# cggos/ptam_cg

Measured on AMD Instinct MI355X. Metric: BA LM iterations/s (50 KF x 5k pts) [+ tracked frames/s @640x480 in 'tracking'], higher is better.
Workload: dtype f64; 1 GPU; bundle_50kf_x_5000pts_dense; keyframes=50, points_total=5000, measurements_total=250000, measurements_rank0=250000, estimator=Tukey, parallelism=1 GPU, halfsample=R

## Files before the change

ptam_cg_amd/csrc/ldlt_chain.inc:

```
struct ChainLds {
    double PF[2][2][NB][6];
    double T0[NB * LDP];
    double T1[NB * LDP];
    double T2[NB * LDP];
    double T3[NB * LDP];
    double T4[NB * LDP];
    double iD[NB], Dv[NB], z[NB];
    double zp[8][NB];
    int one_xcd;
    int staged[2];
};
#define CH_TS (NB * LDP)
#define CH_MAX_NB 28
#define CH_LDS_MAX (160 * 1024)
__host__ __device__ __forceinline__ size_t ch_lds_bytes(int band) { return sizeof(ChainLds) + 8 + (size_t)(band + 1) * CH_TS * sizeof(double); }
#define CH_BW_SL 12
__host__ __device__ __forceinline__ size_t ch_lds_bytes_bw(int band, int nblk) {
    const size_t rhs = (size_t)(2 + CH_BW_SL) * nblk * NB + NB, tiles = (size_t)(band + 1) * CH_TS;
    return sizeof(ChainLds) + 8 + (rhs > tiles ? rhs : tiles) * sizeof(double);
}
#define CH_BW_MAXT 9

__device__ __forceinline__ double ch_ld(const double* p) {
    return __longlong_as_double(__hip_atomic_load((const long long*)p, __ATOMIC_RELAXED, __HIP_MEMORY_SCOPE_AGENT));
}
__device__ __forceinline__ void ch_st(double* p, double v, bool one_xcd) {
    if (one_xcd)
        *p = v;
    else
        __hip_atomic_store((long long*)p, __double_as_longlong(v), __ATOMIC_RELAXED, __HIP_MEMORY_SCOPE_AGENT);
}
__device__ __forceinline__ void ch_ld2_issue(double2& v, const double2* p) { asm volatile("global_load_dwordx4 %0, %1, off sc1" : "=v"(v) : "v"(p) : "memory"); }
__device__ __forceinline__ void ch_ld2_wait() { asm volatile("s_waitcnt vmcnt(0)" ::: "memory"); }
__device__ __forceinline__ void ch_raise(unsigned* f, unsigned seq, bool one_xcd) {
    const unsigned v = (seq << 1) | (one_xcd ? 1u : 0u);
    if (one_xcd)
        asm volatile("global_store_dword %0, %1, off" ::"v"(f), "v"(v) : "memory");
    else
        __hip_atomic_store(f, v, __ATOMIC_RELAXED, __HIP_MEMORY_SCOPE_AGENT);
}
__device__ __forceinline__ unsigned ch_flag(const unsigned* f) { return __hip_atomic_load(f, __ATOMIC_RELAXED, __HIP_MEMORY_SCOPE_AGENT); }
__device__ __forceinline__ unsigned ch_wait(const unsigned* f, unsigned seq, unsigned* err, int limit) {
    int spins = 0;
    unsigned v;
    while (((v = ch_flag(f)) >> 1) != seq) {
        __builtin_amdgcn_s_sleep(1);
        if (++spins > limit || ((spins & 255) == 0 && ch_flag(err) == seq)) {
            __hip_atomic_store(err, seq, __ATOMIC_RELAXED, __HIP_MEMORY_SCOPE_AGENT);
            break;
        }
    }
    return v;
}
__device__ __forceinline__ void ch_wait_lanes(const unsigned* f, bool active, unsigned seq, unsigned* err, int limit) {
    int spins = 0;
    for (;;) {
        const bool up = !active || (ch_flag(f) >> 1) == seq;
        if (__builtin_amdgcn_ballot_w64(!up) == 0) break;
        __builtin_amdgcn_s_sleep(1);
        if (++spins > limit || ((spins & 255) == 0 && ch_flag(err) == seq)) {
            __hip_atomic_store(err, seq, __ATOMIC_RELAXED, __HIP_MEMORY_SCOPE_AGENT);
            break;
        }
    }
}
__host__ __device__ __forceinline__ int ch_roles(int nblk) { return nblk > 2 ? nblk : 2; }
__host__ __device__ __forceinline__ size_t ch_flag_words(int nblk, int band) { return 2 + 3 * (size_t)nblk + (size_t)nblk * (band + 1); }

struct ChainArgs {
    double *S, *E, *L, *Dg, *y;
    unsigned* flags;
    int k0, k1, kr, n;
};
__global__ void __launch_bounds__(TPB, 2) ldlt_chain_kernel(BaDev d, ChainArgs a0, ChainArgs a1, int clubs, int cur, int do_bw) {
    const int club = ((int)(blockIdx.x & 7) - d.chain_xcd) & 7;
    if (club >= clubs) return;
    const ChainArgs& a = club == 0 ? a0 : a1;
    const int k0 = a.k0, k1 = a.k1, kr = a.kr;
    const int role = blockIdx.x >> 3;
    if (role == 0 && club == 0) { TL_MARK(d, 9) }
    extern __shared__ __attribute__((aligned(16))) double ch_lds[];
    ChainLds& s = *(ChainLds*)ch_lds;
    const int band = se_band(d), nblk = d.npad / NB;
    const int n_roles = ch_roles(kr - k0);
    if (role >= n_roles) return;
    const unsigned seq = d.solve_seq;
    unsigned* const err = d.sflags;
    unsigned* const F = a.flags + 1;
    unsigned* const RF = F + nblk;
    unsigned* const XCC = RF + nblk;
    unsigned* const XFb = XCC + nblk + 1;
    auto XF = [&](int r, int m) { return XFb + (size_t)r * (band + 1) + (m - max(0, r - band)); };
    double* __restrict__ S = a.S;
    double* __restrict__ E = a.E;
    double* __restrict__ Lf = a.L;
    const int tid = threadIdx.x;
    const int w = __builtin_amdgcn_readfirstlane(tid >> 6), lane = tid & 63;
    const int qi = w >> 1, qj = w & 1;
    const int i16 = lane & 15, m4 = lane >> 4;
    const int colq = 16 * qj + i16;
    const unsigned my_xcc = __builtin_amdgcn_s_getreg(20 | (0 << 6) | (3 << 11)) & 0xf;
    if (tid == 0) __hip_atomic_store(XCC + role, (seq << 4) | my_xcc, __ATOMIC_RELAXED, __HIP_MEMORY_SCOPE_AGENT);
    auto mma_t = [&](const double* A, const double (&bt)[NB / 4]) {
        v4f64 acc = {0, 0, 0, 0};
        const double* pa = A + (16 * qi + i16) * LDP + m4;
        double a8[NB / 4];
#pragma unroll
        for (int kk = 0; kk < NB / 4; kk++) a8[kk] = pa[4 * kk];
#pragma unroll
        for (int kk = 0; kk < NB / 4; kk++) acc = __builtin_amdgcn_mfma_f64_16x16x4f64(a8[kk], bt[kk], acc, 0, 0, 0);
        return acc;
    };
#ifdef K7_TIMING
    int nst_ = 0;
#define CH_STAMP() if (role == 0 && threadIdx.x == 192 && nst_ < 200) d.dbg[32 + nst_++] = (long long)__builtin_readcyclecounter();
#define CH_SEEN(t_) if (lane == 0) d.dbg[440 + k] = d.dbg[456 + k] = 100 + (t_);
#define CH_RT(slot) d.dbg[600 + (slot)] = (long long)__builtin_amdgcn_s_memrealtime();
#else
#define CH_STAMP()
#define CH_SEEN(t_)
#define CH_RT(slot)
#endif
    if (role == 0) {
        const double e0 = m4 == 0 ? 1.0 : 0.0, e1 = m4 == 1 ? 1.0 : 0.0, e2 = m4 == 2 ? 1.0 : 0.0, e3 = m4 == 3 ? 1.0 : 0.0;
        v4f64 accK;
#pragma unroll
        for (int v = 0; v < 4; v++) {
            const int row = 16 * qi + m4 + 4 * v;
            accK[v] = S[se_blk(k0, k0, band) + max(row, colq) * NB + min(row, colq)];
        }
        bool one_xcd = false;
        for (int k = k0; k < k1; k++) {
            v4f64 accI;
            const int niter = (min(NB, a.n - k * NB) + 3) / 4;
            if (tid < NB) {
                s.iD[tid] = 1.0;
                s.Dv[tid] = 1.0;
            }
            const int r = k + 1;
            const bool have_row = r < kr;
            const size_t o_rk = have_row ? se_blk(r, k, band) : 0, o_rr = have_row ? se_blk(r, r, band) : 0;
            if (tid < 2) s.staged[tid] = 0;
            int stage_state = have_row ? 0 : 2;
            double stg[2][NB * NB / 64];
            CH_STAMP()
            if (tid == 0) { CH_RT(4 * k + 3) }
#ifdef FL_NO_STAGE
#define FL_STAGE_ON false
#else
#define FL_STAGE_ON true
#endif
#define FACTOR_IDLE_HOOK(t_)                                                                                         \
    if (FL_STAGE_ON && stage_state < 2) {                                                                            \
        if (stage_state == 0 && (r < k0 + 2 || (ch_flag(RF + r) >> 1) == seq)) {                                     \
            _Pragma("unroll") for (int u = 0; u < NB * NB / 64; u++) stg[0][u] = ch_ld(S + o_rk + lane + 64 * u);    \
            _Pragma("unroll") for (int u = 0; u < NB * NB / 64; u++) stg[1][u] = ch_ld(S + o_rr + lane + 64 * u);    \
            stage_state = (t_) + 1 < niter ? 1 : 3;                                                                  \
            CH_SEEN(t_)                                                                                              \
        } else if (stage_state == 1)                                                                                 \
            stage_state = 3;                                                                                         \
        if (stage_state == 3) {                                                                                      \
            _Pragma("unroll") for (int u = 0; u < NB * NB / 64; u++) {                                               \
                const int e_ = lane + 64 * u;                                                                        \
                s.T3[(e_ / NB) * LDP + e_ % NB] = stg[0][u];                                                         \
                s.T4[(e_ / NB) * LDP + e_ % NB] = stg[1][u];                                                         \
            }                                                                                                        \
            if (lane == 0) s.staged[0] = s.staged[1] = 1;                                                            \
            stage_state = 2;                                                                                         \
        }                                                                                                            \
    }
#include "ldlt_factor2.inc"
#undef FACTOR_IDLE_HOOK
            CH_STAMP()
            if (k == k0) {
                if (w == 0) {
                    bool same = true;
                    for (int i = lane; i < n_roles; i += 64) same = same && ch_flag(XCC + i) == ((seq << 4) | my_xcc);
                    const bool all_same = __builtin_amdgcn_ballot_w64(!same) == 0;
                    if (lane == 0) s.one_xcd = all_same;
                }
                __syncthreads();
                one_xcd = s.one_xcd != 0;
            }
            const size_t o_kk = se_blk(k, k, band);
#pragma unroll
            for (int v = 0; v < 4; v++)
                s.T0[(16 * qi + m4 + 4 * v) * LDP + fl_colI] = accI[v];
            auto store_diag = [&]() {
#pragma unroll
                for (int v = 0; v < 4; v++) ch_st(Lf + o_kk + (16 * qi + m4 + 4 * v) * NB + fl_colI, accI[v], one_xcd);
                if (tid < NB) ch_st(a.Dg + k * NB + tid, s.Dv[tid], one_xcd);
            };
            if (!have_row) {
                store_diag();
                asm volatile("s_waitcnt vmcnt(0)" ::: "memory");
                __syncthreads();
                if (tid == 0) ch_raise(F + k, seq, one_xcd);
                break;
            }
            double aop[NB / 4];
            v4f64 accN;
            if (!(s.staged[0] && s.staged[1])) {
                if (r >= k0 + 2 && lane == 0) ch_wait(RF + r, seq, err, d.spin_limit);
                double t3[NB * NB / TPB], t4[NB * NB / TPB];
#pragma unroll
                for (int u = 0; u < NB * NB / TPB; u++) t3[u] = ch_ld(S + o_rk + tid + u * TPB);
#pragma unroll
                for (int u = 0; u < NB * NB / TPB; u++) t4[u] = ch_ld(S + o_rr + tid + u * TPB);
#pragma unroll
                for (int u = 0; u < NB * NB / TPB; u++) {
                    const int e = tid + u * TPB;
                    s.T3[(e / NB) * LDP + e % NB] = t3[u];
                    s.T4[(e / NB) * LDP + e % NB] = t4[u];
                }
                __syncthreads();
            }
#pragma unroll
            for (int kk = 0; kk < NB / 4; kk++) aop[kk] = s.T3[(16 * qi + i16) * LDP + 4 * kk + m4];
#pragma unroll
            for (int v = 0; v < 4; v++) {
                const int row = 16 * qi + m4 + 4 * v;
                accN[v] = s.T4[max(row, colq) * LDP + min(row, colq)];
            }
            CH_STAMP()
            __syncthreads();
            v4f64 x = {0, 0, 0, 0};
            {
                const double* pb = s.T0 + m4 * LDP + colq;
                double b8[NB / 4];
#pragma unroll
                for (int kk = 0; kk < NB / 4; kk++) b8[kk] = pb[4 * kk * LDP];
#pragma unroll
                for (int kk = 0; kk < NB / 4; kk++) x = __builtin_amdgcn_mfma_f64_16x16x4f64(aop[kk], b8[kk], x, 0, 0, 0);
            }
            const double idc = s.iD[colq];
            __builtin_amdgcn_sched_barrier(0);
            store_diag();
            __builtin_amdgcn_sched_barrier(0);
            double lv[4];
#pragma unroll
            for (int v = 0; v < 4; v++) {
                const int e = (16 * qi + m4 + 4 * v);
                lv[v] = x[v] * idc;
                s.T1[e * LDP + colq] = x[v];
                s.T2[e * LDP + colq] = lv[v];
            }
            __syncthreads();
            double bt[NB / 4];
#pragma unroll
            for (int kk = 0; kk < NB / 4; kk++) bt[kk] = s.T2[(16 * qj + i16) * LDP + 4 * kk + m4];
            const v4f64 upd = mma_t(s.T1, bt);
            __builtin_amdgcn_sched_barrier(0);
#pragma unroll
            for (int v = 0; v < 4; v++) ch_st(Lf + o_rk + (16 * qi + m4 + 4 * v) * NB + colq, lv[v], one_xcd);
            __builtin_amdgcn_sched_barrier(0);
#pragma unroll
            for (int v = 0; v < 4; v++) accK[v] = accN[v] - upd[v];
            asm volatile("s_waitcnt vmcnt(0)" ::: "memory");
            __syncthreads();
            if (tid == 0) {
                ch_raise(F + k, seq, one_xcd);
                ch_raise(XF(r, k), seq, one_xcd);
                CH_RT(4 * k)
            }
            if (r == k1) {
                if (w != 1) {
#pragma unroll
                    for (int v = 0; v < 4; v++) S[o_rr + (16 * qi + m4 + 4 * v) * NB + colq] = accK[v];
                }
                break;
            }
            CH_STAMP()
        }
        return;
    }
    if (role == n_roles - 1) {
        double* const bb = ch_lds + (sizeof(ChainLds) + 7) / 8;
        const int b0 = k0 * NB;
        for (int i = k0 * NB + tid; i < kr * NB; i += TPB) bb[i - b0] = E[i];
        __syncthreads();
        const int q = tid & (NB - 1), part = tid >> 5;
        const int row = tid >> 3, g = tid & 7;
        for (int m = k0; m < k1; m++) {
            if (lane == 0) (void)ch_wait(F + m, seq, err, d.spin_limit);
            const size_t o_mm = se_blk(m, m, band);
            double t4[NB / 8];
#pragma unroll
            for (int j = 0; j < NB / 8; j++) t4[j] = ch_ld(Lf + o_mm + (part + 8 * j) * NB + q);
            double p = 0;
#pragma unroll
            for (int j = 0; j < NB / 8; j++) p += t4[j] * bb[m * NB - b0 + part + 8 * j];
            s.zp[part][q] = p;
            __syncthreads();
            if (tid < NB) {
                const double z = ((s.zp[0][tid] + s.zp[1][tid]) + (s.zp[2][tid] + s.zp[3][tid])) +
                                 ((s.zp[4][tid] + s.zp[5][tid]) + (s.zp[6][tid] + s.zp[7][tid]));
                s.z[tid] = z;
                a.y[m * NB + tid] = z;
                if (do_bw) bb[m * NB - b0 + tid] = z / ch_ld(a.Dg + m * NB + tid);
            }
            __syncthreads();
            double zr[NB / 8];
#pragma unroll
            for (int jj = 0; jj < NB / 8; jj++) zr[jj] = s.z[g + 8 * jj];
            const int jhi = min(kr - 1, m + band);
            {
                const int jw = m + 1 + lane;
                ch_wait_lanes(XF(min(jw, jhi), m), jw <= jhi && jhi > m, seq, err, d.spin_limit);
            }
            for (int jb = m + 1; jb <= jhi; jb += 4) {
                const int nj = min(4, jhi - jb + 1);
                double lv[4][NB / 8];
#pragma unroll
                for (int u = 0; u < 4; u++)
                    if (u < nj) {
                        const double* Lj = Lf + se_blk(jb + u, m, band) + row * NB + g;
#pragma unroll
                        for (int jj = 0; jj < NB / 8; jj++) lv[u][jj] = ch_ld(Lj + 8 * jj);
                    }
#pragma unroll
                for (int u = 0; u < 4; u++)
                    if (u < nj) {
                        double sum = 0;
#pragma unroll
                        for (int jj = 0; jj < NB / 8; jj++) sum += lv[u][jj] * zr[jj];
                        sum += dpp_row_shr_f64<1>(sum);
                        sum += dpp_row_shr_f64<2>(sum);
                        sum += dpp_row_shr_f64<4>(sum);
                        if (g == 7) bb[(jb + u) * NB - b0 + row] -= sum;
                    }
            }
            __syncthreads();
        }
        for (int i = k1 * NB + tid; i < kr * NB; i += TPB) E[i] = bb[i - b0];
        if (!do_bw) return;
        {
            const int nrow = kr * NB;
            double* const xs = bb + nrow;
            double* const pend = xs + nrow;
            for (int i = tid; i < CH_BW_SL * nrow; i += TPB) pend[i] = 0.0;
            const int hh = lane >> 5, c32 = lane & (NB - 1);
            const int g4 = lane >> 4, cp = lane & 15;
            constexpr int TW = 3;
            static_assert(3 * TW >= CH_BW_MAXT, "three tile waves cover a block row");
            static_assert(CH_BW_SL == 12, "a slice per tile wave and lane group");
            const int tw = w - 1;
            double* const dstage0 = s.T1;
            static_assert(4 * NB * LDP >= 2 * NB * 34, "the diagonal tiles' staging areas");
            auto stage_diag = [&](int k) {
                const double2* dk = (const double2*)(Lf + se_blk(k, k, band)) + lane;
                double2 dq[3];
#pragma unroll
                for (int i = 0; i < 3; i++)
                    if (tw + 3 * i < NB / 4) ch_ld2_issue(dq[i], dk + 64 * (tw + 3 * i));
                ch_ld2_wait();
                double* const ds = dstage0 + (k & 1) * (NB * 34);
#pragma unroll
                for (int i = 0; i < 3; i++)
                    if (tw + 3 * i < NB / 4) *(double2*)(ds + (4 * (tw + 3 * i) + g4) * 34 + 2 * cp) = dq[i];
            };
            if (w > 0) stage_diag(kr - 1);
            __syncthreads();
#ifdef K7_TIMING
#define BWI_STAMP(i_) if (lane == 0 && w < 2) d.dbg[1400 + 8 * k + 4 * w + (i_)] = (long long)__builtin_readcyclecounter();
            if (tid == 0) d.dbg[1399] = (long long)__builtin_readcyclecounter();
#else
#define BWI_STAMP(i_)
#endif
#pragma unroll 1
            for (int k = kr - 1; k >= 0; k--) {
                const int jb0 = max(0, k - band), nt = k - jb0;
                BWI_STAMP(0)
                double2 lt[TW][NB / 4];
                if (w == 0) {
                    const double* pk = pend + k * NB + c32;
                    const double v = bb[k * NB + c32] - ((((pk[0] + pk[nrow]) + (pk[2 * nrow] + pk[3 * nrow])) + ((pk[4 * nrow] + pk[5 * nrow]) + (pk[6 * nrow] + pk[7 * nrow]))) +
                                                         ((pk[8 * nrow] + pk[9 * nrow]) + (pk[10 * nrow] + pk[11 * nrow])));
                    if (hh == 0) s.z[c32] = v;
                    __builtin_amdgcn_fence(__ATOMIC_RELEASE, "wavefront");
                    __builtin_amdgcn_wave_barrier();
                    double tk[NB / 2], zk[NB / 2];
#pragma unroll
                    for (int u = 0; u < NB / 2; u++) tk[u] = dstage0[(k & 1) * (NB * 34) + c32 * 34 + 16 * hh + u], zk[u] = s.z[16 * hh + u];
                    double p4[4] = {0, 0, 0, 0};
#pragma unroll
                    for (int u = 0; u < NB / 2; u++) p4[u & 3] += (16 * hh + u >= c32) ? tk[u] * zk[u] : 0.0;
                    const double p = (p4[0] + p4[1]) + (p4[2] + p4[3]);
                    const unsigned long long pb_ = (unsigned long long)__double_as_longlong(p);
                    const auto lo_ = __builtin_amdgcn_permlane32_swap((unsigned)pb_, (unsigned)pb_, false, false);
                    const auto hi_ = __builtin_amdgcn_permlane32_swap((unsigned)(pb_ >> 32), (unsigned)(pb_ >> 32), false, false);
                    const double p_up = __longlong_as_double((long long)(((unsigned long long)hi_[1] << 32) | lo_[1]));
                    if (hh == 0) xs[k * NB + c32] = p + p_up;
                    BWI_STAMP(1)
                } else {
                    const double2* src = (const double2*)(Lf + se_blk(k, jb0, band)) + lane;
#pragma unroll
                    for (int i = 0; i < TW; i++)
                        if (tw + 3 * i < nt) {
#pragma unroll
                            for (int u = 0; u < NB / 4; u++) ch_ld2_issue(lt[i][u], src + (size_t)(tw + 3 * i) * (NB * NB / 2) + 64 * u);
                        }
                    if (k > 0)
                        stage_diag(k - 1);
                    else
                        ch_ld2_wait();
                }
                BWI_STAMP(2)
                __syncthreads();
                BWI_STAMP(3)
                if (w > 0) {
                    double xv[NB / 4];
#pragma unroll
                    for (int u = 0; u < NB / 4; u++) xv[u] = xs[k * NB + 4 * u + g4];
                    double* const pslot = pend + (4 * tw + g4) * nrow + jb0 * NB + 2 * cp;
#pragma unroll
                    for (int i = 0; i < TW; i++)
                        if (tw + 3 * i < nt) {
                            double a0 = 0, a1 = 0;
#pragma unroll
                            for (int u = 0; u < NB / 4; u++) a0 += lt[i][u].x * xv[u], a1 += lt[i][u].y * xv[u];
                            __hip_atomic_fetch_add(pslot + (tw + 3 * i) * NB, a0, __ATOMIC_RELAXED, __HIP_MEMORY_SCOPE_WORKGROUP);
                            __hip_atomic_fetch_add(pslot + (tw + 3 * i) * NB + 1, a1, __ATOMIC_RELAXED, __HIP_MEMORY_SCOPE_WORKGROUP);
                        }
                }
                __syncthreads();
            }
            __syncthreads();
            for (int i = tid; i < nrow; i += TPB) d.da[i] = xs[i];
            for (int c2 = tid; c2 < d.C; c2 += TPB) {
                const int f = d.cam_free[c2];
                const double* T = d.pose[cur] + 12 * c2;
                double* Tn = d.pose[cur ^ 1] + 12 * c2;
                double Tl[12], o[12];
#pragma unroll
                for (int i = 0; i < 12; i++) Tl[i] = T[i];
                if (f < 0) {
#pragma unroll
                    for (int i = 0; i < 12; i++) Tn[i] = Tl[i];
                } else {
                    double mu[6];
#pragma unroll
                    for (int i = 0; i < 6; i++) mu[i] = xs[6 * f + i];
                    se3_exp_mul(mu, Tl, o);
#pragma unroll
                    for (int i = 0; i < 12; i++) Tn[i] = o[i];
                }
            }
#ifdef K7_TIMING
            if (tid == 0) d.dbg[1398] = (long long)__builtin_readcyclecounter();
#endif
            if (tid < 64) {
                double sq = 0;
                for (int i = tid; i < min(nrow, d.n); i += 64) sq += xs[i] * xs[i];
                sq = wave_sum_f64(sq);
                if (tid == 0) {
                    d.sumsq2[0] = sq;
                    d.sumsq2[1] = 0.0;
                    if (ch_flag(err) != 0) {
                        d.sc->solve_fault = 1;
                        __hip_atomic_store(err, 0u, __ATOMIC_RELAXED, __HIP_MEMORY_SCOPE_AGENT);
                    }
                }
            }
        }
        return;
    }
    const int r = k0 + role + 1;
    if (r >= kr) return;
    const int j0 = max(k0, r - band), nt = r - j0 + 1;
    double* const tiles = ch_lds + (sizeof(ChainLds) + 7) / 8;
    for (int t = 0; t < nt; t++) {
        const size_t o = se_blk(r, j0 + t, band);
        double v4[NB * NB / TPB];
#pragma unroll
        for (int u = 0; u < NB * NB / TPB; u++) v4[u] = S[o + tid + u * TPB];
#pragma unroll
        for (int u = 0; u < NB * NB / TPB; u++) {
            const int e = tid + u * TPB;
            tiles[t * CH_TS + (e / NB) * LDP + e % NB] = v4[u];
        }
    }
    __syncthreads();
    bool one_xcd = false, stored_direct = false;
    const int m_last = min(r - 2, k1 - 1);
    for (int m = j0; m <= m_last; m++) {
        unsigned fv = 0;
        if (lane == 0) fv = ch_wait(F + m, seq, err, d.spin_limit);
        one_xcd = (__builtin_amdgcn_readfirstlane(fv) & 1u) != 0;
        if (tid == 0 && m == r - 2) { CH_RT(4 * m + 1) }
        if (tid == 0 && r == k1 - 1) { CH_RT(100 + 4 * m) }
        const size_t o_mm = se_blk(m, m, band), o_rm = se_blk(r, m, band);
        double lm[NB / 4], ln[NB * NB / TPB];
#pragma unroll
        for (int kk = 0; kk < NB / 4; kk++) lm[kk] = ch_ld(Lf + o_mm + (4 * kk + m4) * NB + colq);
        const double dgc = ch_ld(a.Dg + m * NB + colq);
        {
            const double* Lj = Lf + se_blk(m + 1, m, band) + tid;
#pragma unroll
            for (int i = 0; i < NB * NB / TPB; i++) ln[i] = ch_ld(Lj + TPB * i);
        }
        const double* tA = tiles + (m - j0) * CH_TS + (16 * qi + i16) * LDP + m4;
        double a8[NB / 4];
#pragma unroll
        for (int kk = 0; kk < NB / 4; kk++) a8[kk] = tA[4 * kk];
        v4f64 x = {0, 0, 0, 0};
#pragma unroll
        for (int kk = 0; kk < NB / 4; kk++) x = __builtin_amdgcn_mfma_f64_16x16x4f64(a8[kk], lm[kk], x, 0, 0, 0);
        const double idc = fast_rcp(dgc);
#pragma unroll
        for (int v = 0; v < 4; v++) {
            const int e = (16 * qi + m4 + 4 * v);
            const double l = x[v] * idc;
            ch_st(Lf + o_rm + e * NB + colq, l, one_xcd);
            s.T1[e * LDP + colq] = x[v];
            s.T2[e * LDP + colq] = l;
        }
#pragma unroll
        for (int i = 0; i < NB * NB / TPB; i++) {
            const int e = tid + TPB * i;
            s.T3[(e / NB) * LDP + e % NB] = ln[i];
        }
        const bool last_pivot = m == m_last;
        if (!last_pivot) asm volatile("s_waitcnt vmcnt(0)" ::: "memory");
        __syncthreads();
        if (tid == 0 && !last_pivot) ch_raise(XF(r, m), seq, one_xcd);
        if (tid == 0 && r == k1 - 1) { CH_RT(100 + 4 * m + 1) }
        const bool to_S = last_pivot && m == r - 2;
        auto update = [&](int j, const double (&bt)[NB / 4]) {
            const v4f64 upd = mma_t(s.T1, bt);
            double* tj = tiles + (j - j0) * CH_TS + (16 * qi + m4) * LDP + colq;
            double* gj = S + se_blk(r, j, band) + (16 * qi + m4) * NB + colq;
#pragma unroll
            for (int v = 0; v < 4; v++) {
                const double nv = tj[4 * v * LDP] - upd[v];
                tj[4 * v * LDP] = nv;
                if (to_S) ch_st(gj + 4 * v * NB, nv, one_xcd);
            }
        };
        stored_direct = to_S;
        {
            double bt1[NB / 4];
#pragma unroll
            for (int kk = 0; kk < NB / 4; kk++) bt1[kk] = s.T3[(16 * qj + i16) * LDP + 4 * kk + m4];
            update(m + 1, bt1);
        }
        {
            double btr[NB / 4];
#pragma unroll
            for (int kk = 0; kk < NB / 4; kk++) btr[kk] = s.T2[(16 * qj + i16) * LDP + 4 * kk + m4];
            update(r, btr);
        }
        if (tid == 0 && r == k1 - 1) { CH_RT(100 + 4 * m + 2) }
        {
            const int jw = m + 2 + lane;
            ch_wait_lanes(XF(min(jw, nblk - 1), m), jw < r, seq, err, d.spin_limit);
        }
        {
            constexpr int RT = 3;
            double* const stage[RT] = {s.T0, s.T3, s.T4};
            auto issue = [&](int jb, double (&pr)[RT][NB * NB / TPB]) {
#pragma unroll
                for (int u = 0; u < RT; u++)
                    if (jb + u < r) {
                        const double* src = Lf + se_blk(jb + u, m, band) + tid;
#pragma unroll
                        for (int i = 0; i < NB * NB / TPB; i++) pr[u][i] = ch_ld(src + TPB * i);
                    }
            };
            auto round = [&](int jb, const double (&cur)[RT][NB * NB / TPB], double (&nxt)[RT][NB * NB / TPB]) {
                if (jb + RT < r) issue(jb + RT, nxt);
#pragma unroll
                for (int u = 0; u < RT; u++)
                    if (jb + u < r) {
#pragma unroll
                        for (int i = 0; i < NB * NB / TPB; i++) {
                            const int e = tid + TPB * i;
                            stage[u][(e / NB) * LDP + e % NB] = cur[u][i];
                        }
                    }
                __syncthreads();
#pragma unroll
                for (int u = 0; u < RT; u++)
                    if (jb + u < r) {
                        double bt[NB / 4];
#pragma unroll
                        for (int kk = 0; kk < NB / 4; kk++) bt[kk] = stage[u][(16 * qj + i16) * LDP + 4 * kk + m4];
                        update(jb + u, bt);
                    }
                __syncthreads();
            };
            double pa[RT][NB * NB / TPB], pb[RT][NB * NB / TPB];
            if (m + 2 < r) {
                issue(m + 2, pa);
                __syncthreads();
            }
            for (int jb = m + 2; jb < r; jb += 2 * RT) {
                round(jb, pa, pb);
                if (jb + RT < r) round(jb + RT, pb, pa);
            }
        }
        __syncthreads();
        if (tid == 0 && r == k1 - 1) { CH_RT(100 + 4 * m + 3) }
    }
    {
        const int jf = max(j0, min(r - 1, k1));
        if (m_last < j0) one_xcd = false;
        for (int j = jf; j <= r && !stored_direct; j++) {
            const size_t o = se_blk(r, j, band);
            const double* tj = tiles + (j - j0) * CH_TS;
#pragma unroll
            for (int e = tid; e < NB * NB; e += TPB) ch_st(S + o + e, tj[(e / NB) * LDP + e % NB], one_xcd);
        }
        asm volatile("s_waitcnt vmcnt(0)" ::: "memory");
        __syncthreads();
        if (tid == 0) {
            if (m_last >= j0) ch_raise(XF(r, m_last), seq, one_xcd);
            ch_raise(RF + r, seq, one_xcd);
            CH_RT(4 * (r - 2) + 2)
        }
    }
}

__global__ void __launch_bounds__(TPB) ldlt_mirror_in_kernel(BaDev d, int kr) {
    const int band = se_band(d), nblk = d.npad / NB;
    const int bi = blockIdx.x / (band + 1), jo = blockIdx.x % (band + 1), bj = bi - band + jo;
    if (bi >= kr || bj < 0) return;
    const double* __restrict__ src = d.SE + se_blk(nblk - 1 - bj, nblk - 1 - bi, band);
    double* __restrict__ dst = d.SE2 + se_blk(bi, bj, band);
    double v[NB * NB / TPB];
#pragma unroll
    for (int i = 0; i < NB * NB / TPB; i++) v[i] = src[threadIdx.x + TPB * i];
#pragma unroll
    for (int i = 0; i < NB * NB / TPB; i++) {
        const int e = threadIdx.x + TPB * i;
        const int a = e / NB, b = e % NB;
        dst[(NB - 1 - b) * NB + (NB - 1 - a)] = v[i];
    }
    if (bi == bj && threadIdx.x < NB)
        d.SE2[se_size(nblk, band) + bi * NB + threadIdx.x] = se_E(d)[(nblk - 1 - bi) * NB + NB - 1 - threadIdx.x];
}
__global__ void __launch_bounds__(TPB) ldlt_mirror_out_kernel(BaDev d, int k1, int kr) {
    const int band = se_band(d), nblk = d.npad / NB;
    const int bi = blockIdx.x / (band + 1), jo = blockIdx.x % (band + 1), bj = bi - band + jo;
    if (bi >= kr || bj < 0) return;
    const int pi = nblk - 1 - bi, pj = nblk - 1 - bj;
    const int tid = threadIdx.x;
    if (bj < k1) {
        const double* __restrict__ src = d.L2 + se_blk(bi, bj, band);
        double v[NB * NB / TPB];
#pragma unroll
        for (int i = 0; i < NB * NB / TPB; i++) v[i] = src[tid + TPB * i];
        if (bi == bj) {
            double* __restrict__ dst = d.L + se_blk(pi, pi, band);
#pragma unroll
            for (int i = 0; i < NB * NB / TPB; i++) dst[tid + TPB * i] = v[i];
            if (tid < NB) {
                d.Dg[pi * NB + tid] = d.Dg2[bi * NB + tid];
                d.y[pi * NB + tid] = d.y2[bi * NB + tid];
            }
        } else {
            double* __restrict__ dst = d.L + se_blk(pj, pi, band);
#pragma unroll
            for (int i = 0; i < NB * NB / TPB; i++) {
                const int e = tid + TPB * i;
                const int r = e / NB, q = e % NB;
                dst[q * NB + (NB - 1 - r)] = v[i];
            }
        }
    } else {
        const double* __restrict__ src = d.SE2 + se_blk(bi, bj, band);
        double* __restrict__ dst = d.SE + se_blk(pj, pi, band);
        double v[NB * NB / TPB];
#pragma unroll
        for (int i = 0; i < NB * NB / TPB; i++) v[i] = src[tid + TPB * i];
#pragma unroll
        for (int i = 0; i < NB * NB / TPB; i++) {
            const int e = tid + TPB * i;
            const int r = e / NB, c = e % NB;
            dst[(NB - 1 - c) * NB + (NB - 1 - r)] = v[i];
        }
        if (bi == bj && tid < NB) se_E(d)[pi * NB + NB - 1 - tid] = d.SE2[se_size(nblk, band) + bi * NB + tid];
    }
}
```

ptam_cg_amd/csrc/solve.hip:

```cpp
#include "bundle.h"

#define NB SOLVE_NB
#define LDP (NB + 1)
#define STRIPS 8
#define CPT (NB / STRIPS)
#define TPB (NB * STRIPS)
#define NITER (NB / 4)
#define BW_LDS_MAX ((size_t)150 * 1024)
static_assert(NB == 32, "the strip decomposition below is written for 32x32 blocks");

__device__ __forceinline__ double fast_rcp(double d) {
    const double y = __builtin_amdgcn_rcp(d);
    const double e = fma(-d, y, 1.0);
    return fma(y, fma(e, e, e), y);
}

struct Micro {
    double l10, l20, l21, l30, l31, l32;
    double i0, i1, i2, i3;
    double d0, d1, d2, d3, u10, u20, u30, u21, u31, u32;
};
__device__ __forceinline__ Micro micro_factor(double m00, double m10, double m11, double m20, double m21, double m22,
                                              double m30, double m31, double m32, double m33) {
    Micro f;
    f.d0 = m00;
    f.u10 = m10;
    f.u20 = m20;
    f.u30 = m30;
    f.i0 = fast_rcp(m00);
    f.l10 = m10 * f.i0;
    f.l20 = m20 * f.i0;
    f.l30 = m30 * f.i0;
    f.d1 = m11 - f.l10 * m10;
    f.i1 = fast_rcp(f.d1);
    f.u21 = m21 - f.l20 * m10;
    f.u31 = m31 - f.l30 * m10;
    f.l21 = f.u21 * f.i1;
    f.l31 = f.u31 * f.i1;
    f.d2 = m22 - f.l20 * m20 - f.l21 * f.u21;
    f.i2 = fast_rcp(f.d2);
    f.u32 = m32 - f.l30 * m20 - f.l31 * f.u21;
    f.l32 = f.u32 * f.i2;
    f.d3 = m33 - f.l30 * m30 - f.l31 * f.u31 - f.l32 * f.u32;
    f.i3 = fast_rcp(f.d3);
    return f;
}
__device__ __forceinline__ void micro_subst(const Micro& f, const double a[4], double x[4]) {
    x[0] = a[0];
    x[1] = a[1] - x[0] * f.l10;
    x[2] = a[2] - x[0] * f.l20 - x[1] * f.l21;
    x[3] = a[3] - x[0] * f.l30 - x[1] * f.l31 - x[2] * f.l32;
}

typedef double v4f64 __attribute__((ext_vector_type(4)));
struct StepLds {
    double P[2][3][NB][4];
    double Pb[2][4];
    double Xi[NB * LDP];
    double Xj[NB * LDP];
    double iD[NB], Dv[NB], z[NB];
};

__global__ void __launch_bounds__(TPB) ldlt_step_kernel(BaDev d, int k, int row_limit) {
    if (k == 0) { TL_MARK(d, 9) }
    __shared__ StepLds s;
    constexpr bool mir = false;
    const int wg = blockIdx.x;
    const int rem = min(row_limit - k - 1, se_band(d));
#include "ldlt_step_body.inc"
}

__global__ void __launch_bounds__(TPB) ldlt_step_twin_kernel(BaDev d, int k_top, int k_bot, int nwg_top) {
    if (k_top == 0) { TL_MARK(d, 9) }
    __shared__ StepLds s;
    if ((int)blockIdx.x >= nwg_top) {
        constexpr bool mir = true;
        const int k = k_bot, wg = (int)blockIdx.x - nwg_top;
        const int rem = min(k, se_band(d));
#include "ldlt_step_body.inc"
    } else {
        constexpr bool mir = false;
        const int k = k_top, wg = blockIdx.x;
        const int rem = min(d.npad / NB - k - 1, se_band(d));
#include "ldlt_step_body.inc"
    }
}

#include "ldlt_small.inc"
#include "ldlt_chain.inc"

template <bool BIG>
__global__ void __launch_bounds__(1024) ldlt_backward_kernel(BaDev d, int cur, int b_start) {
    TL_MARK(d, 10)
    const int chain = blockIdx.x;
    extern __shared__ __attribute__((aligned(16))) double bw_lds[];
    const int npad = d.npad, nblk = npad / NB, band = se_band(d);
    double* xs = BIG ? d.bw_scratch + (size_t)chain * 6 * npad : bw_lds;
    double* pend = xs + npad;
    double* wv = pend + 4 * npad;
    const int tid = threadIdx.x;
    const int c = tid % NB, rr = tid / NB;
    if (tid == 0 && chain == 0 && d.sflags && d.sflags[0] != 0) {
        d.sc->solve_fault = 1;
        d.sflags[0] = 0;
    }
    for (int i = tid; i < npad; i += 1024) {
        pend[i] = pend[npad + i] = pend[2 * npad + i] = pend[3 * npad + i] = 0.0;
        wv[i] = d.y[i] / d.Dg[i];
    }
    const int t_end = nblk - b_start;
    const int k_stop = chain == 0 ? 0 : t_end;
    double wnext = d.L[se_blk(b_start - 1, b_start - 1, band) + rr * NB + c];
#ifdef K7_TIMING
#define BW_STAMP(i) if (tid == 0 && chain == 0) d.dbg[1000 + 8 * k + (i)] = (long long)__builtin_readcyclecounter();
#else
#define BW_STAMP(i)
#endif
    const int ucol = tid & (NB - 1), sl0 = (tid >> 5) & 3, ut0 = tid >> 7;
    auto fetch_l = [&](int k, double (&l)[8]) {
        const int jb0 = max(0, k - band);
        const double* src = d.L + se_blk(k, jb0, band) + (size_t)ut0 * (NB * NB) + (sl0 * 8) * NB + ucol;
        const bool on = ut0 < k - jb0;
#pragma unroll
        for (int q = 0; q < 8; q++) l[q] = on ? src[q * NB] : 0.0;
    };
    for (int k = b_start - 1; k >= k_stop; k--) {
        const double w = wnext;
        if (k > k_stop) wnext = d.L[se_blk(k - 1, k - 1, band) + rr * NB + c];
        double lreg[8];
        fetch_l(k, lreg);
        const int jb0 = max(0, k - band), nbk = k - jb0, jlo = jb0 * NB;
        const double* Lrow = d.L + se_blk(k, jb0, band);
        const bool upd = ut0 < nbk;
        const int j0 = jlo + ut0 * NB + ucol;
        BW_STAMP(0)
        __syncthreads();
        BW_STAMP(1)
        const int kc = k * NB + c;
        double p = (c >= rr) ? w * (wv[kc] - ((pend[kc] + pend[npad + kc]) + (pend[2 * npad + kc] + pend[3 * npad + kc]))) : 0.0;
        p += dpp_row_shr_f64<1>(p);
        p += dpp_row_shr_f64<2>(p);
        p += dpp_row_shr_f64<4>(p);
        p += dpp_row_shr_f64<8>(p);
        p += dpp_bcast_f64<0x142, 0xA>(p);
        if (c == NB - 1) xs[k * NB + rr] = p;
        BW_STAMP(2)
        __syncthreads();
        BW_STAMP(3)
        if (upd) {
            double a = 0;
#pragma unroll
            for (int q = 0; q < 8; q++) a += lreg[q] * xs[k * NB + sl0 * 8 + q];
            pend[sl0 * npad + j0] += a;
        }
        for (int ut = ut0 + 8; ut < nbk; ut += 8) {
            double a = 0;
#pragma unroll
            for (int q = 0; q < 8; q++) a += Lrow[(size_t)ut * (NB * NB) + (sl0 * 8 + q) * NB + ucol] * xs[k * NB + sl0 * 8 + q];
            pend[sl0 * npad + jlo + ut * NB + ucol] += a;
        }
        BW_STAMP(4)
    }
    __syncthreads();
    for (int k = b_start; k < nblk && chain == 1; k++) {
        const int jb = max(0, k - band), nj = k - jb;
        const double w = d.L[se_blk(k, k, band) + rr * NB + c];
        const double* Lrow = d.L + se_blk(k, jb, band) + rr * NB + c;
        double a = 0;
        for (int j = 0; j < nj; j++) a += Lrow[(size_t)j * (NB * NB)] * xs[(jb + j) * NB + c];
        a += dpp_row_shr_f64<1>(a);
        a += dpp_row_shr_f64<2>(a);
        a += dpp_row_shr_f64<4>(a);
        a += dpp_row_shr_f64<8>(a);
        a += dpp_bcast_f64<0x142, 0xA>(a);
        if (c == NB - 1) pend[k * NB + rr] = a;
        __syncthreads();
        const int kc = k * NB + c;
        double p = (c >= rr) ? w * (wv[kc] - pend[kc]) : 0.0;
        p += dpp_row_shr_f64<1>(p);
        p += dpp_row_shr_f64<2>(p);
        p += dpp_row_shr_f64<4>(p);
        p += dpp_row_shr_f64<8>(p);
        p += dpp_bcast_f64<0x142, 0xA>(p);
        if (c == NB - 1) xs[k * NB + (NB - 1 - rr)] = p;
        __syncthreads();
    }
    const bool two = t_end > 0;
    const int r_lo = chain == 0 ? 0 : b_start * NB, r_hi = (two && chain == 0) ? b_start * NB : npad;
    for (int i = r_lo + tid; i < r_hi; i += 1024) d.da[i] = xs[i];
    for (int c2 = tid; c2 < d.C; c2 += 1024) {
        const int f = d.cam_free[c2];
        const bool mine = (two && f >= 0 && 6 * f + 5 >= b_start * NB) ? chain == 1 : chain == 0;
        if (!mine) continue;
        const double* T = d.pose[cur] + 12 * c2;
        double* Tn = d.pose[cur ^ 1] + 12 * c2;
        double Tl[12], o[12];
#pragma unroll
        for (int i = 0; i < 12; i++) Tl[i] = T[i];
        if (f < 0) {
#pragma unroll
            for (int i = 0; i < 12; i++) Tn[i] = Tl[i];
        } else {
            double mu[6];
#pragma unroll
            for (int i = 0; i < 6; i++) mu[i] = xs[6 * f + i];
            se3_exp_mul(mu, Tl, o);
#pragma unroll
            for (int i = 0; i < 12; i++) Tn[i] = o[i];
        }
    }
    if (tid < 64) {
        double sq = 0;
        for (int i = r_lo + tid; i < min(r_hi, d.n); i += 64) sq += xs[i] * xs[i];
        sq = wave_sum_f64(sq);
        if (tid == 0) {
            d.sumsq2[chain] = sq;
            if (!two) d.sumsq2[1] = 0.0;
        }
    }
}

int ba_solve_init() {
    HIP_TRY(hipFuncSetAttribute((const void*)ldlt_backward_kernel<false>, hipFuncAttributeMaxDynamicSharedMemorySize, 160 * 1024));
    HIP_TRY(hipFuncSetAttribute((const void*)ldlt_small_kernel, hipFuncAttributeMaxDynamicSharedMemorySize, 160 * 1024));
    HIP_TRY(hipFuncSetAttribute((const void*)ldlt_chain_kernel, hipFuncAttributeMaxDynamicSharedMemorySize, 160 * 1024));
    return PTAM_OK;
}

static int ldlt_twist_len(int nblk, int band) {
    static const bool off = ptam_ab_env("PTAM_LDLT_ONE_ENDED") != nullptr;
    if (off || band < 1 || nblk < 2 * band + 8) return 0;
    return (nblk - 2 * band) / 2;
}

size_t ba_solve_flag_bytes(int nblk) { return ch_flag_words(nblk, nblk) * sizeof(unsigned); }

static ChainArgs chain_args_natural(const BaDev& d, int k0, int k1, int kr) {
    return ChainArgs{d.SE, se_E(d), d.L, d.Dg, d.y, d.sflags, k0, k1, kr, d.n};
}

int ba_solve(ptam_ctx* ctx, BaDev& d, int cur) {
    const int nblk = d.npad / NB, band = se_band(d);
    static const bool no_small = ptam_ab_env("PTAM_LDLT_NO_SMALL") != nullptr;
    if (!no_small && nblk <= SM_USE_NB) {
        hipLaunchKernelGGL(ldlt_small_kernel, dim3(1), dim3(TPB), sizeof(SmallLds), ctx->stream, d, cur);
        HIP_TRY(hipGetLastError());
        return PTAM_OK;
    }
    auto nwg_of = [](int rem) { return 1 + rem + rem * (rem + 1) / 2; };
    const int t_end = ldlt_twist_len(nblk, band), b_start = nblk - t_end;
    {
        static const bool no_chain = getenv("PTAM_LDLT_NO_CHAIN") != nullptr;
        static const bool sep_bw = getenv("PTAM_LDLT_SEPARATE_BACKWARD") != nullptr;
        const bool bw_in = !sep_bw && band <= CH_BW_MAXT && ch_lds_bytes_bw(band, nblk) <= CH_LDS_MAX;
        const size_t lds = bw_in ? ch_lds_bytes_bw(band, nblk) : ch_lds_bytes(band);
        if (t_end == 0 && !no_chain && !d.chain_off && d.sflags && nblk <= CH_MAX_NB && lds <= CH_LDS_MAX) {
            d.solve_seq++;
            if (d.solve_seq >= (1u << 27)) d.solve_seq = 1;
            {
                const ChainArgs a = chain_args_natural(d, 0, nblk, nblk);
                hipLaunchKernelGGL(ldlt_chain_kernel, dim3(8 * ch_roles(nblk)), dim3(TPB), lds, ctx->stream, d, a, a, 1, cur, bw_in ? 1 : 0);
            }
            if (!bw_in) {
                const size_t bw = (size_t)6 * d.npad * sizeof(double);
                hipLaunchKernelGGL(ldlt_backward_kernel<false>, dim3(1), dim3(1024), bw, ctx->stream, d, cur, nblk);
            }
            HIP_TRY(hipGetLastError());
            return PTAM_OK;
        }
    }
    static const bool no_chain2 = getenv("PTAM_LDLT_NO_CHAIN") != nullptr || ptam_ab_env("PTAM_LDLT_TWIN_LAUNCHES") != nullptr;
    const int kr2 = std::min(b_start, t_end + band);
    const bool two_persistent = t_end >= 2 && !no_chain2 && !d.chain_off && d.sflags && d.SE2 && kr2 <= CH_MAX_NB && ch_lds_bytes(band) <= CH_LDS_MAX;
    if (two_persistent) {
        d.solve_seq++;
        if (d.solve_seq >= (1u << 27)) d.solve_seq = 1;
        hipLaunchKernelGGL(ldlt_mirror_in_kernel, dim3(kr2 * (band + 1)), dim3(TPB), 0, ctx->stream, d, kr2);
        const ChainArgs a0 = chain_args_natural(d, 0, t_end, kr2);
        const ChainArgs a1{d.SE2, d.SE2 + se_size(nblk, band), d.L2, d.Dg2, d.y2, d.sflags2, 0, t_end, kr2, d.npad};
        hipLaunchKernelGGL(ldlt_chain_kernel, dim3(8 * ch_roles(kr2)), dim3(TPB), ch_lds_bytes(band), ctx->stream, d, a0, a1, 2, cur, 0);
        hipLaunchKernelGGL(ldlt_mirror_out_kernel, dim3(kr2 * (band + 1)), dim3(TPB), 0, ctx->stream, d, t_end, kr2);
    }
    for (int st = 0; st < (two_persistent ? 0 : t_end); st++) {
        const int kt = st, kb = nblk - 1 - st;
        const int nt = nwg_of(std::min(nblk - kt - 1, band)), nb = nwg_of(std::min(kb, band));
        hipLaunchKernelGGL(ldlt_step_twin_kernel, dim3(nt + nb), dim3(TPB), 0, ctx->stream, d, kt, kb, nt);
    }
    {
        static const bool no_chain = getenv("PTAM_LDLT_NO_CHAIN") != nullptr;
        const int n_mid = b_start - t_end;
        const size_t lds = ch_lds_bytes(band);
        if (t_end > 0 && !no_chain && !d.chain_off && d.sflags && n_mid >= 3 && n_mid <= CH_MAX_NB && lds <= CH_LDS_MAX) {
            d.solve_seq++;
            if (d.solve_seq >= (1u << 27)) d.solve_seq = 1;
            {
                const ChainArgs a = chain_args_natural(d, t_end, b_start, b_start);
                hipLaunchKernelGGL(ldlt_chain_kernel, dim3(8 * ch_roles(n_mid)), dim3(TPB), lds, ctx->stream, d, a, a, 1, cur, 0);
            }
        } else {
            for (int k = t_end; k < b_start; k++) {
                const int nwg = nwg_of(std::min(b_start - k - 1, band));
                hipLaunchKernelGGL(ldlt_step_kernel, dim3(nwg), dim3(TPB), 0, ctx->stream, d, k, b_start);
            }
        }
    }
    const size_t bw_bytes = (size_t)6 * d.npad * sizeof(double);
    if (bw_bytes > BW_LDS_MAX)
        hipLaunchKernelGGL(ldlt_backward_kernel<true>, dim3(t_end > 0 ? 2 : 1), dim3(1024), 0, ctx->stream, d, cur, b_start);
    else
        hipLaunchKernelGGL(ldlt_backward_kernel<false>, dim3(t_end > 0 ? 2 : 1), dim3(1024), bw_bytes, ctx->stream, d, cur, b_start);
    HIP_TRY(hipGetLastError());
    return PTAM_OK;
}

void solve_preload_kernels() {
    ptam_preload((const void*)ldlt_step_kernel);
    ptam_preload((const void*)ldlt_step_twin_kernel);
    ptam_preload((const void*)ldlt_backward_kernel<false>);
    ptam_preload((const void*)ldlt_backward_kernel<true>);
    ptam_preload((const void*)ldlt_small_kernel);
    ptam_preload((const void*)ldlt_chain_kernel);
    ptam_preload((const void*)ldlt_mirror_in_kernel);
    ptam_preload((const void*)ldlt_mirror_out_kernel);
}
```

Measured before the change: 6375 LM iterations/s.

## Overlap backward substitution with factorization via per-column inverse-block workgroups

Adds a forward-inverse mode to the chained LDLT kernel for small block counts. Extra workgroups, one per block column, build columns of L^{-T} as factor tiles arrive and take dot products with the forward-solve scaled results, publishing solution slices through flags. The serial backward substitution at the end is replaced by a gather and the pose update. It trades extra MFMA work, more workgroups, LDS use and flag traffic for a shorter critical path after factorization.

```diff
diff --git a/ptam_cg_amd/csrc/ldlt_chain.inc b/ptam_cg_amd/csrc/ldlt_chain.inc
--- a/ptam_cg_amd/csrc/ldlt_chain.inc
+++ b/ptam_cg_amd/csrc/ldlt_chain.inc
@@ -19,6 +19,10 @@
     const size_t rhs = (size_t)(2 + CH_BW_SL) * nblk * NB + NB, tiles = (size_t)(band + 1) * CH_TS;
     return sizeof(ChainLds) + 8 + (rhs > tiles ? rhs : tiles) * sizeof(double);
 }
+__host__ __device__ __forceinline__ size_t ch_lds_bytes_fi(int band, int nblk) {
+    return sizeof(ChainLds) + 8 + (size_t)(band + 1 > nblk ? band + 1 : nblk) * CH_TS * sizeof(double);
+}
+#define CH_FI_MAX_NB 13
 #define CH_BW_MAXT 9
 
 __device__ __forceinline__ double ch_ld(const double* p) {
@@ -65,7 +69,8 @@
     }
 }
 __host__ __device__ __forceinline__ int ch_roles(int nblk) { return nblk > 2 ? nblk : 2; }
-__host__ __device__ __forceinline__ size_t ch_flag_words(int nblk, int band) { return 2 + 3 * (size_t)nblk + (size_t)nblk * (band + 1); }
+__host__ __device__ __forceinline__ int ch_roles_fi(int nblk) { return ch_roles(nblk) + nblk; }
+__host__ __device__ __forceinline__ size_t ch_flag_words(int nblk, int band) { return 2 + 6 * (size_t)nblk + (size_t)nblk * (band + 1); }
 
 struct ChainArgs {
     double *S, *E, *L, *Dg, *y;
@@ -83,13 +88,17 @@
     ChainLds& s = *(ChainLds*)ch_lds;
     const int band = se_band(d), nblk = d.npad / NB;
     const int n_roles = ch_roles(kr - k0);
-    if (role >= n_roles) return;
+    const int n_col = do_bw == 2 ? kr - k0 : 0;
+    if (role >= n_roles + n_col) return;
     const unsigned seq = d.solve_seq;
     unsigned* const err = d.sflags;
     unsigned* const F = a.flags + 1;
     unsigned* const RF = F + nblk;
     unsigned* const XCC = RF + nblk;
     unsigned* const XFb = XCC + nblk + 1;
+    unsigned* const WF = XFb + (size_t)nblk * (band + 1);
+    unsigned* const XD = WF + nblk;
+    unsigned* const XCC2 = XD + nblk;
     auto XF = [&](int r, int m) { return XFb + (size_t)r * (band + 1) + (m - max(0, r - band)); };
     double* __restrict__ S = a.S;
     double* __restrict__ E = a.E;
@@ -100,7 +109,7 @@
     const int i16 = lane & 15, m4 = lane >> 4;
     const int colq = 16 * qj + i16;
     const unsigned my_xcc = __builtin_amdgcn_s_getreg(20 | (0 << 6) | (3 << 11)) & 0xf;
-    if (tid == 0) __hip_atomic_store(XCC + role, (seq << 4) | my_xcc, __ATOMIC_RELAXED, __HIP_MEMORY_SCOPE_AGENT);
+    if (tid == 0) __hip_atomic_store(role < n_roles ? XCC + role : XCC2 + (role - n_roles), (seq << 4) | my_xcc, __ATOMIC_RELAXED, __HIP_MEMORY_SCOPE_AGENT);
     auto mma_t = [&](const double* A, const double (&bt)[NB / 4]) {
         v4f64 acc = {0, 0, 0, 0};
         const double* pa = A + (16 * qi + i16) * LDP + m4;
@@ -175,7 +184,7 @@
             if (k == k0) {
                 if (w == 0) {
                     bool same = true;
-                    for (int i = lane; i < n_roles; i += 64) same = same && ch_flag(XCC + i) == ((seq << 4) | my_xcc);
+                    for (int i = lane; i < n_roles + n_col; i += 64) same = same && ch_flag(i < n_roles ? XCC + i : XCC2 + (i - n_roles)) == ((seq << 4) | my_xcc);
                     const bool all_same = __builtin_amdgcn_ballot_w64(!same) == 0;
                     if (lane == 0) s.one_xcd = all_same;
                 }
@@ -195,7 +204,10 @@
                 store_diag();
                 asm volatile("s_waitcnt vmcnt(0)" ::: "memory");
                 __syncthreads();
-                if (tid == 0) ch_raise(F + k, seq, one_xcd);
+                if (tid == 0) {
+                    ch_raise(F + k, seq, one_xcd);
+                    CH_RT(200)
+                }
                 break;
             }
             double aop[NB / 4];
@@ -282,7 +294,10 @@
         const int q = tid & (NB - 1), part = tid >> 5;
         const int row = tid >> 3, g = tid & 7;
         for (int m = k0; m < k1; m++) {
-            if (lane == 0) (void)ch_wait(F + m, seq, err, d.spin_limit);
+            unsigned fv = 0;
+            if (lane == 0) fv = ch_wait(F + m, seq, err, d.spin_limit);
+            const bool one_xcd = (__builtin_amdgcn_readfirstlane(fv) & 1u) != 0;
+            if (tid == 0 && m == k1 - 1) { CH_RT(201) }
             const size_t o_mm = se_blk(m, m, band);
             double t4[NB / 8];
 #pragma unroll
@@ -296,8 +311,16 @@
                 const double z = ((s.zp[0][tid] + s.zp[1][tid]) + (s.zp[2][tid] + s.zp[3][tid])) +
                                  ((s.zp[4][tid] + s.zp[5][tid]) + (s.zp[6][tid] + s.zp[7][tid]));
                 s.z[tid] = z;
-                a.y[m * NB + tid] = z;
-                if (do_bw) bb[m * NB - b0 + tid] = z / ch_ld(a.Dg + m * NB + tid);
+                if (do_bw != 2) a.y[m * NB + tid] = z;
+                if (do_bw == 1) bb[m * NB - b0 + tid] = z / ch_ld(a.Dg + m * NB + tid);
+                if (do_bw == 2) ch_st(d.bw_scratch + m * NB + tid, z / ch_ld(a.Dg + m * NB + tid), one_xcd);
+            }
+            if (do_bw == 2 && w == 0) {
+                asm volatile("s_waitcnt vmcnt(0)" ::: "memory");
+                if (lane == 0) {
+                    ch_raise(WF + m, seq, one_xcd);
+                    if (m == k1 - 1) { CH_RT(202) }
+                }
             }
             __syncthreads();
             double zr[NB / 8];
@@ -334,6 +357,54 @@
         }
         for (int i = k1 * NB + tid; i < kr * NB; i += TPB) E[i] = bb[i - b0];
         if (!do_bw) return;
+        auto finish = [&](const double* xs, int nrow) {
+            for (int c2 = tid; c2 < d.C; c2 += TPB) {
+                const int f = d.cam_free[c2];
+                const double* T = d.pose[cur] + 12 * c2;
+                double* Tn = d.pose[cur ^ 1] + 12 * c2;
+                double Tl[12], o[12];
+#pragma unroll
+                for (int i = 0; i < 12; i++) Tl[i] = T[i];
+                if (f < 0) {
+#pragma unroll
+                    for (int i = 0; i < 12; i++) Tn[i] = Tl[i];
+                } else {
+                    double mu[6];
+#pragma unroll
+                    for (int i = 0; i < 6; i++) mu[i] = xs[6 * f + i];
+                    se3_exp_mul(mu, Tl, o);
+#pragma unroll
+                    for (int i = 0; i < 12; i++) Tn[i] = o[i];
+                }
+            }
+#ifdef K7_TIMING
+            if (tid == 0) d.dbg[1398] = (long long)__builtin_readcyclecounter();
+#endif
+            if (tid < 64) {
+                double sq = 0;
+                for (int i = tid; i < min(nrow, d.n); i += 64) sq += xs[i] * xs[i];
+                sq = wave_sum_f64(sq);
+                if (tid == 0) {
+                    d.sumsq2[0] = sq;
+                    d.sumsq2[1] = 0.0;
+                    if (ch_flag(err) != 0) {
+                        d.sc->solve_fault = 1;
+                        __hip_atomic_store(err, 0u, __ATOMIC_RELAXED, __HIP_MEMORY_SCOPE_AGENT);
+                    }
+                }
+            }
+        };
+        if (do_bw == 2) {
+            const int nrow = kr * NB;
+            double* const xs = bb + nrow;
+            ch_wait_lanes(XD + min(lane, kr - 1), lane < kr, seq, err, d.spin_limit);
+            if (tid == 0) { CH_RT(207) }
+            for (int i = tid; i < nrow; i += TPB) xs[i] = ch_ld(d.da + i);
+            __syncthreads();
+            finish(xs, nrow);
+            if (tid == 0) { CH_RT(208) }
+            return;
+        }
         {
             const int nrow = kr * NB;
             double* const xs = bb + nrow;
@@ -427,40 +498,109 @@
             }
             __syncthreads();
             for (int i = tid; i < nrow; i += TPB) d.da[i] = xs[i];
-            for (int c2 = tid; c2 < d.C; c2 += TPB) {
-                const int f = d.cam_free[c2];
-                const double* T = d.pose[cur] + 12 * c2;
-                double* Tn = d.pose[cur ^ 1] + 12 * c2;
-                double Tl[12], o[12];
-#pragma unroll
-                for (int i = 0; i < 12; i++) Tl[i] = T[i];
-                if (f < 0) {
-#pragma unroll
-                    for (int i = 0; i < 12; i++) Tn[i] = Tl[i];
-                } else {
-                    double mu[6];
-#pragma unroll
-                    for (int i = 0; i < 6; i++) mu[i] = xs[6 * f + i];
-                    se3_exp_mul(mu, Tl, o);
-#pragma unroll
-                    for (int i = 0; i < 12; i++) Tn[i] = o[i];
-                }
-            }
-#ifdef K7_TIMING
-            if (tid == 0) d.dbg[1398] = (long long)__builtin_readcyclecounter();
-#endif
-            if (tid < 64) {
-                double sq = 0;
-                for (int i = tid; i < min(nrow, d.n); i += 64) sq += xs[i] * xs[i];
-                sq = wave_sum_f64(sq);
-                if (tid == 0) {
-                    d.sumsq2[0] = sq;
-                    d.sumsq2[1] = 0.0;
-                    if (ch_flag(err) != 0) {
-                        d.sc->solve_fault = 1;
-                        __hip_atomic_store(err, 0u, __ATOMIC_RELAXED, __HIP_MEMORY_SCOPE_AGENT);
-                    }
-                }
+            finish(xs, nrow);
+        }
+        return;
+    }
+    if (role >= n_roles) {
+        const int j = role - n_roles;
+        double* const Rt = ch_lds + (sizeof(ChainLds) + 7) / 8;
+        for (int e = tid; e < (kr - j) * CH_TS; e += TPB) Rt[e] = 0.0;
+        __syncthreads();
+        if (tid < NB) Rt[tid * LDP + tid] = 1.0;
+        __syncthreads();
+        const int c32 = tid & (NB - 1), part = tid >> 5;
+        double xp = 0;
+        bool one_xcd = false;
+        for (int m = j; m < kr; m++) {
+            unsigned fv = 0;
+            if (lane == 0) fv = ch_wait(F + m, seq, err, d.spin_limit);
+            one_xcd = (__builtin_amdgcn_readfirstlane(fv) & 1u) != 0;
+            if (tid == 0 && j == 0 && m == kr - 1) { CH_RT(203) }
+            {
+                const double* Tm = Lf + se_blk(m, m, band) + m4 * NB + 16 * qi + i16;
+                const double* Rm = Rt + (m - j) * CH_TS + m4 * LDP + colq;
+                double a8[NB / 4], b8[NB / 4];
+#pragma unroll
+                for (int kk = 0; kk < NB / 4; kk++) a8[kk] = ch_ld(Tm + 4 * kk * NB);
+#pragma unroll
+                for (int kk = 0; kk < NB / 4; kk++) b8[kk] = Rm[4 * kk * LDP];
+                v4f64 y = {0, 0, 0, 0};
+#pragma unroll
+                for (int kk = 0; kk < NB / 4; kk++) y = __builtin_amdgcn_mfma_f64_16x16x4f64(a8[kk], b8[kk], y, 0, 0, 0);
+#pragma unroll
+                for (int v = 0; v < 4; v++) s.T2[(16 * qi + m4 + 4 * v) * LDP + colq] = y[v];
+            }
+            __syncthreads();
+            if (tid == 0 && j == 0 && m == kr - 1) { CH_RT(204) }
+            const int jhi = min(kr - 1, m + band);
+            if (jhi > m) {
+                {
+                    const int jw = m + 1 + lane;
+                    ch_wait_lanes(XF(min(jw, jhi), m), jw <= jhi, seq, err, d.spin_limit);
+                }
+                double bt[NB / 4];
+#pragma unroll
+                for (int kk = 0; kk < NB / 4; kk++) bt[kk] = s.T2[(4 * kk + m4) * LDP + colq];
+                constexpr int RT = 3;
+                double* const stage[RT] = {s.T0, s.T3, s.T4};
+                auto issue = [&](int jb, double (&pr)[RT][NB * NB / TPB]) {
+#pragma unroll
+                    for (int u = 0; u < RT; u++)
+                        if (jb + u <= jhi) {
+                            const double* src = Lf + se_blk(jb + u, m, band) + tid;
+#pragma unroll
+                            for (int i = 0; i < NB * NB / TPB; i++) pr[u][i] = ch_ld(src + TPB * i);
+                        }
+                };
+                auto round = [&](int jb, const double (&now)[RT][NB * NB / TPB], double (&nxt)[RT][NB * NB / TPB]) {
+                    if (jb + RT <= jhi) issue(jb + RT, nxt);
+#pragma unroll
+                    for (int u = 0; u < RT; u++)
+                        if (jb + u <= jhi) {
+#pragma unroll
+                            for (int i = 0; i < NB * NB / TPB; i++) {
+                                const int e = tid + TPB * i;
+                                stage[u][(e / NB) * LDP + e % NB] = now[u][i];
+                            }
+                        }
+                    __syncthreads();
+#pragma unroll
+                    for (int u = 0; u < RT; u++)
+                        if (jb + u <= jhi) {
+                            const v4f64 upd = mma_t(stage[u], bt);
+                            double* rj = Rt + (jb + u - j) * CH_TS + (16 * qi + m4) * LDP + colq;
+#pragma unroll
+                            for (int v = 0; v < 4; v++) rj[4 * v * LDP] -= upd[v];
+                        }
+                    __syncthreads();
+                };
+                double pa[RT][NB * NB / TPB], pb[RT][NB * NB / TPB];
+                issue(m + 1, pa);
+                for (int jb = m + 1; jb <= jhi; jb += 2 * RT) {
+                    round(jb, pa, pb);
+                    if (jb + RT <= jhi) round(jb + RT, pb, pa);
+                }
+            }
+            if (lane == 0) (void)ch_wait(WF + m, seq, err, d.spin_limit);
+            if (tid == 0 && j == 0 && m == kr - 1) { CH_RT(205) }
+            double wv[NB / 8];
+#pragma unroll
+            for (int jj = 0; jj < NB / 8; jj++) wv[jj] = ch_ld(d.bw_scratch + m * NB + part + 8 * jj);
+#pragma unroll
+            for (int jj = 0; jj < NB / 8; jj++) xp += s.T2[(part + 8 * jj) * LDP + c32] * wv[jj];
+            __syncthreads();
+        }
+        s.zp[part][c32] = xp;
+        __syncthreads();
+        if (w == 0) {
+            if (tid < NB)
+                ch_st(d.da + j * NB + tid,
+                      ((s.zp[0][tid] + s.zp[1][tid]) + (s.zp[2][tid] + s.zp[3][tid])) + ((s.zp[4][tid] + s.zp[5][tid]) + (s.zp[6][tid] + s.zp[7][tid])), one_xcd);
+            asm volatile("s_waitcnt vmcnt(0)" ::: "memory");
+            if (lane == 0) {
+                ch_raise(XD + j, seq, one_xcd);
+                if (j == 0) { CH_RT(206) }
             }
         }
         return;
diff --git a/ptam_cg_amd/csrc/solve.hip b/ptam_cg_amd/csrc/solve.hip
--- a/ptam_cg_amd/csrc/solve.hip
+++ b/ptam_cg_amd/csrc/solve.hip
@@ -233,6 +233,12 @@
     return (nblk - 2 * band) / 2;
 }
 
+static bool ldlt_forward_inverse(int nblk, int band) {
+    static const bool off = getenv("PTAM_LDLT_BACKWARD_IN_LAUNCH") != nullptr || getenv("PTAM_LDLT_SEPARATE_BACKWARD") != nullptr ||
+                            getenv("PTAM_LDLT_NO_CHAIN") != nullptr;
+    return !off && ldlt_twist_len(nblk, band) == 0 && nblk > SM_USE_NB && nblk <= CH_FI_MAX_NB && ch_lds_bytes_fi(band, nblk) <= CH_LDS_MAX;
+}
+
 size_t ba_solve_flag_bytes(int nblk) { return ch_flag_words(nblk, nblk) * sizeof(unsigned); }
 
 static ChainArgs chain_args_natural(const BaDev& d, int k0, int k1, int kr) {
@@ -253,15 +259,17 @@
         static const bool no_chain = getenv("PTAM_LDLT_NO_CHAIN") != nullptr;
         static const bool sep_bw = getenv("PTAM_LDLT_SEPARATE_BACKWARD") != nullptr;
         const bool bw_in = !sep_bw && band <= CH_BW_MAXT && ch_lds_bytes_bw(band, nblk) <= CH_LDS_MAX;
-        const size_t lds = bw_in ? ch_lds_bytes_bw(band, nblk) : ch_lds_bytes(band);
+        const bool fwd_inv = ldlt_forward_inverse(nblk, band);
+        const int do_bw = fwd_inv ? 2 : bw_in ? 1 : 0;
+        const size_t lds = fwd_inv ? ch_lds_bytes_fi(band, nblk) : bw_in ? ch_lds_bytes_bw(band, nblk) : ch_lds_bytes(band);
         if (t_end == 0 && !no_chain && !d.chain_off && d.sflags && nblk <= CH_MAX_NB && lds <= CH_LDS_MAX) {
             d.solve_seq++;
             if (d.solve_seq >= (1u << 27)) d.solve_seq = 1;
             {
                 const ChainArgs a = chain_args_natural(d, 0, nblk, nblk);
-                hipLaunchKernelGGL(ldlt_chain_kernel, dim3(8 * ch_roles(nblk)), dim3(TPB), lds, ctx->stream, d, a, a, 1, cur, bw_in ? 1 : 0);
+                hipLaunchKernelGGL(ldlt_chain_kernel, dim3(8 * (fwd_inv ? ch_roles_fi(nblk) : ch_roles(nblk))), dim3(TPB), lds, ctx->stream, d, a, a, 1, cur, do_bw);
             }
-            if (!bw_in) {
+            if (!do_bw) {
                 const size_t bw = (size_t)6 * d.npad * sizeof(double);
                 hipLaunchKernelGGL(ldlt_backward_kernel<false>, dim3(1), dim3(1024), bw, ctx->stream, d, cur, nblk);
             }
```

After: 6812 LM iterations/s (median of 6 runs). +6.9%, better.
